# Genomics-GPU/Genomics-GPU

Hardware: AMD Instinct MI355X
Metric: GCUPS on batched 150bp affine-gap SW at 1/2/4/8 MI355X; HBM-roofline % (higher is better)
Workload: dtype int16x2 packed (exact value window), int32 fallback per declined block

## Files before the change

genomics-gpu_amd/csrc/dispatch.hip:

```cpp
#include <hip/hip_runtime.h>

#include <algorithm>
#include <cstdio>
#include <cstdlib>
#include <cstring>
#include <string>
#include <vector>

#include "banded16.hpp"
#include "local16.hpp"
#include "engine.hpp"
#include "generic.hpp"
#include "pairhmm.hpp"
#include "ksw16.hpp"
#include "start.hpp"
#include "wavefront.hpp"
#include "wavefront16.hpp"

namespace gx {

static thread_local std::string g_last_error;
void set_error(const std::string &msg) { g_last_error = msg; }
const char *last_error() { return g_last_error.c_str(); }

// ... 339 lines not shown
    uint32_t b0 = 0, p0 = 0, ppb = 1, lds_stride = 0;
    size_t lds_bytes = 0;
    int32_t vmin = 0;
};
static bool one_shape_only(const WfArgs &A) { return A.rev || A.n_dev || A.stop || A.lstop; }

static int device_cus(Workspace &ws) {
    if (!ws.cus) (void)hipDeviceGetAttribute(&ws.cus, hipDeviceAttributeMultiprocessorCount, ws.device);
    return ws.cus > 0 ? ws.cus : 256;
}

static TailShape tail_shape(Workspace &ws, const Plan &pl, const gasalx_params &p, const WfArgs &A, uint32_t n) {
    TailShape t;
    const bool on = env_flag("GASALX_TAIL", true);
    const int kextra = env_int("GASALX_TAIL_K", 0);
    if (!on || !pl.packed16 || (pl.tb && !pl.tb_band) || pl.key2 || pl.ku16 || pl.kseg_shift || pl.semi_tq ||
        one_shape_only(A))
        return t;
    int G2 = 0, R2 = 0;
    WfFn fn = nullptr;
    if (pl.wf_algo == WF_LOCAL && pl.kf16 && pl.G16 == 8 && pl.R16 == 19) {
        G2 = 32; R2 = 5; fn = &wf16_mix_kernel<WF_LOCAL, 8, 19, 32, 5>;
    } else if (pl.tb_band) {
        if (pl.wf_algo != WF_GLOBAL || pl.G16 != 16 || pl.R16 != 20) return t;
        if (env_int("GASALX_CP_TAIL", 64) == 32) {
            G2 = 32; R2 = 12; fn = &wf16_mix_kernel<WF16_GLOBAL_CP, 16, 20, 32, 12>;
        } else {
            G2 = 64; R2 = 8; fn = &wf16_mix_kernel<WF16_GLOBAL_CP, 16, 20, 64, 8>;
        }
    } else if (pl.wf_algo == WF_GLOBAL && pl.G16 == 16 && pl.R16 == 20) {
        G2 = 64; R2 = 5; fn = &wf16_mix_kernel<WF_GLOBAL, 16, 20, 64, 5>;
    } else {
        return t;
    }
    const int64_t q8 = pad8(pl.max_q), y8 = pad8(pl.max_t);
    if (pl.wf_algo == WF_LOCAL) {
        const LocalDrift d = local_drift_frame(p, q8, y8, G2, R2);
        if (!(d.window && d.f16)) return t;
        t.vmin = pl.vmin;
    } else {
        if (!packed16_ok(p, WF_GLOBAL, pl.max_q, pl.max_t, &t.vmin,
                         std::max(packed_span(G2, R2, y8), packed_span(pl.G16, pl.R16, y8))))
            return t;
        t.vmin = std::max(t.vmin, pl.vmin);
    }
    const uint64_t slots = (uint64_t)wf16_waves(pl.wf_algo, pl.R16) * 4 * device_cus(ws);
    const uint32_t ppw = pairs_per_wave(pl.G16), ppb = pairs_per_block(pl.G16);
    const uint64_t waves = (n + ppw - 1) / ppw;
    const uint64_t rounds = waves / slots;
    if (rounds < 2 + (uint64_t)std::max(kextra, 0)) return t;
    const uint64_t long_waves = (rounds - (uint64_t)std::max(kextra, 0)) * slots;
    t.b0 = (uint32_t)(long_waves / kWavesPerBlock);
    t.p0 = t.b0 * ppb;
    if (t.p0 >= n) return TailShape();
    t.ppb = pairs_per_block(G2);
    t.lds_stride = packed_lds_stride((uint32_t)y8, G2);
    t.lds_bytes = packed_lds_bytes((uint32_t)y8, G2);
    t.fn = fn;
    t.G2 = G2;
    t.R2 = R2;
    return t;
}

template <class Args>
static void fill_scoring(Args &A, const gasalx_params &p) {
    A.a = p.match; A.b = p.mismatch; A.o = p.gap_open; A.e = p.gap_extend;
    A.nval = p.n_code & 0xF;
    A.has_npen = p.has_n_penalty; A.npen = p.n_penalty;
}
static void wf_common(WfArgs &A, const gasalx_params &p, const Plan &pl) {
    fill_scoring(A, p);
    A.head = p.head; A.tail = p.tail;
    A.lds_stride = pl.lds_stride;
    A.force_exact = (p.mismatch <= 0 || (p.has_n_penalty && p.n_penalty < 0)) ? 1 : 0;
    A.one = 0x00010001u;
}

static int launch_int32(const Plan &pl, WfFn fn, const WfArgs &A, hipStream_t st) {
    if (!fn) { set_error("no wavefront instance"); return GASALX_EUNSUPPORTED; }
    HIPCHK(launch_lds(fn, dim3(wf_grid(A.n, pl.G, A.skip != nullptr)), dim3(kBlock), pl.lds_bytes, st, A));
    return GASALX_OK;
}

static int launch_wavefront(Workspace &ws, const Plan &pl, const gasalx_params &p, const WfArgs &base,
                            const TailShape &main_tail, hipStream_t st) {
    WfArgs A = base;
    const uint32_t n = A.n;
    wf_common(A, p, pl);
    if (pl.packed16) {
        WfArgs P16 = A;
        P16.lds_stride = pl.lds16_stride;
        P16.fast16 = 1;
        P16.vmin = pl.vmin;
        P16.kf16 = pl.kf16;
        const uint32_t ppb16 = pairs_per_block(pl.G16);
        uint32_t grid16 = grid_for(n, ppb16);
        const TailShape tail = one_shape_only(A) ? TailShape() : main_tail;
        size_t lds16 = pl.lds16_bytes;
        if (tail.fn) {
            P16.tail_b0 = tail.b0; P16.tail_p0 = tail.p0; P16.tail_lds = tail.lds_stride;
            P16.vmin = tail.vmin;
            grid16 = tail.b0 + grid_for(n - tail.p0, tail.ppb);
            lds16 = std::max(lds16, tail.lds_bytes);
        }
        HIPCHK(ws.misc.reserve(grid16 + 64));
        P16.handled = ws.misc.as<uint8_t>();
        ws.pk_flags = grid16; ws.pk_ppb = ppb16; ws.pk_pairs = n;
        ws.pk_p1 = tail.fn ? tail.p0 : 0xFFFFFFFFu; ws.pk_b1 = tail.b0; ws.pk_ppb2 = tail.fn ? tail.ppb : 1;
        if (pl.tb) {
            HIPCHK(ws.aux.reserve((size_t)n * 4));
            P16.tbfix = ws.aux.as<int32_t>();
        }
        Wf16Variant v;
        v.tb = pl.tb; v.tbd = pl.tb && pl.kf16 != 0;
        v.key2 = pl.key2; v.ku16 = pl.ku16; v.kseg = pl.kseg_shift != 0;
        v.lrs = pl.wf_algo == WF_LOCAL && !pl.tb && !pl.key2 && A.lstop != nullptr && pl.kf16 != 0 && !pl.kseg_shift;
        v.stop = A.stop != nullptr;
        WfFn f16 = pl.tb_band ? wf16_pick_r4<WF16_GLOBAL_CP>(pl.G16, pl.R16) : wf16_lookup(pl.wf_algo, pl.G16, pl.R16, v);
        if (A.rev && !pl.tb_band && (v.stop || v.lrs)) {
            const int ra = A.stop ? WF16_SEMI_STOP : pl.ku16 ? WF16_LOCAL_U16_RS : WF16_LOCAL_RS;
            if (WfFn rc = wf16_rclass_lookup(ra, pl.G16, pl.R16)) f16 = rc;
        }
        if (pl.kseg_shift) {
            const uint32_t nsave = std::max<uint32_t>(1u, (pl.kf16 + (uint32_t)pl.G16 - 2u) >> pl.kseg_shift);
            const uint64_t waves = (uint64_t)grid16 * kWavesPerBlock;
            HIPCHK(ws.kseg.reserve(waves * nsave * (uint64_t)pl.R16 * 64 * 4 + 64));
            P16.kseg = ws.kseg.as<uint32_t>();
            P16.kseg_shift = pl.kseg_shift;
            P16.kseg_n = nsave;
        }
        if (tail.fn) f16 = tail.fn;
        if (!f16) { set_error("no packed wavefront instance"); return GASALX_EUNSUPPORTED; }
        HIPCHK(launch_lds(f16, dim3(grid16), dim3(kBlock), lds16, st, P16));
        A.skip = ws.misc.as<uint8_t>();
        A.skip_ppb = ppb16;
        A.skip_p1 = tail.fn ? tail.p0 : 0xFFFFFFFFu;
        A.skip_b1 = tail.b0;
        A.skip_ppb2 = tail.fn ? tail.ppb : 1;
    }
    return launch_int32(pl, A.stop ? pick_instance<WfK<WF_SEMI, true, false, true>, SHAPES_R4>(pl.G, pl.R)
                                   : wf_lookup(pl.wf_algo, pl.keys, pl.tb && !pl.tb_band, pl.G, pl.R), A, st);
}

struct SortMeta {
    uint32_t *perm, *second, *hist, *cursor;
    size_t sh;
};
static int sort_reserve(Workspace &ws, uint32_t n, uint32_t nkeys, bool two, SortMeta *m) {
    m->sh = (size_t)(nkeys + 1) * 4;
    HIPCHK(ws.sort_meta.reserve((size_t)n * (two ? 8 : 4) + 2 * m->sh + 64));
    m->perm = ws.sort_meta.as<uint32_t>();
    m->second = two ? m->perm + n : nullptr;
    m->hist = m->perm + (two ? 2 : 1) * (size_t)n;
    m->cursor = m->hist + nkeys + 1;
    return GASALX_OK;
}
static int sort_histogram(const SortMeta &m, const uint32_t *keys, uint32_t n, uint32_t nkeys, hipStream_t st) {
    HIPCHK(hipMemsetAsync(m.hist, 0, m.sh, st));
    rev_hist_kernel<<<sort_grid(n), 256, m.sh, st>>>(REV_PLAIN, keys, nullptr, n, nkeys, m.hist);
    HIPCHK(hipGetLastError());
    return GASALX_OK;
}
static int sort_scatter(const SortMeta &m, const uint32_t *keys, uint32_t n, uint32_t nkeys, uint32_t *inv,
                        hipStream_t st) {
    rev_scan_kernel<<<1, 256, 0, st>>>(m.hist, m.cursor, nkeys + 1);
    rev_scatter_kernel<<<sort_grid(n), 256, 2 * m.sh, st>>>(REV_PLAIN, keys, nullptr, n, nkeys, m.cursor, m.perm, inv);
    HIPCHK(hipGetLastError());
    return GASALX_OK;
}
static int counting_sort(Workspace &ws, const uint32_t *keys, uint32_t n, uint32_t nkeys, hipStream_t st,
                         bool want_inv, const uint32_t **perm, const uint32_t **inv) {
    SortMeta m;
    int rc = sort_reserve(ws, n, nkeys, want_inv, &m);
    if (!rc) rc = sort_histogram(m, keys, n, nkeys, st);
    if (!rc) rc = sort_scatter(m, keys, n, nkeys, m.second, st);
    if (rc) return rc;
    *perm = m.perm;
    if (want_inv) *inv = m.second;
    return GASALX_OK;
}

static int launch_semi_tq(Workspace &ws, const Plan &pl, const gasalx_params &p, const WfArgs &base,
                          hipStream_t st, bool one_class) {
    WfArgs A = base;
    const uint32_t n = A.n;
    wf_common(A, p, pl);
    const uint32_t t8w = (uint32_t)pl.R16;
    SortMeta m;
    int rc = sort_reserve(ws, n, t8w, false, &m);
    if (rc) return rc;
    std::vector<uint32_t> h(t8w + 1, 0u);
    if (one_class) {
        h[0] = n;
    } else {
        if ((rc = sort_histogram(m, A.tlen, n, t8w, st))) return rc;
        HIPCHK(hipMemcpyAsync(h.data(), m.hist, m.sh, hipMemcpyDeviceToHost, st));
        HIPCHK(hipStreamSynchronize(st));
    }
    int classes = 0;
    for (uint32_t b = 0; b <= t8w; b++) classes += h[b] != 0;
    A.perm = nullptr;
    if (classes > 1) {
        if ((rc = sort_scatter(m, A.tlen, n, t8w, nullptr, st))) return rc;
        A.perm = m.perm;
    }
    HIPCHK(ws.misc.reserve(n + 64));
    HIPCHK(hipMemsetAsync(ws.misc.p, 0, n, st));
    ws.pk_flags = n; ws.pk_ppb = 1; ws.pk_pairs = n;
    WfArgs P16 = A;
    P16.lds_stride = pl.lds16_stride;
    P16.fast16 = 1;
    P16.vmin = pl.vmin;
    P16.handled = ws.misc.as<uint8_t>();
    const uint32_t ppb16 = pairs_per_block(8);
    uint32_t slot = 0;
    for (uint32_t b = 0; b <= t8w; slot += h[b], b++) {
// ... 611 lines not shown
```

genomics-gpu_amd/csrc/wavefront16.hpp:

```cpp
#pragma once
#include <hip/hip_runtime.h>
#include <stdint.h>

#include <type_traits>

#include "wavefront.hpp"

namespace gx {

typedef unsigned short pk_u2 __attribute__((ext_vector_type(2)));
#define GX_AS(T, x) __builtin_bit_cast(T, x)

__device__ __forceinline__ uint32_t pk_mad_u16(uint32_t a, uint32_t b, uint32_t c) {
    return GX_AS(uint32_t, GX_AS(pk_u2, a) * GX_AS(pk_u2, b) + GX_AS(pk_u2, c));
}
__device__ __forceinline__ uint32_t pk_mad_u16_lo(uint32_t a, uint32_t b, uint32_t c) {
    const pk_u2 cc = {(uint16_t)c, (uint16_t)c};
    return GX_AS(uint32_t, GX_AS(pk_u2, a) * GX_AS(pk_u2, b) + cc);
}
__device__ __forceinline__ uint32_t pk_max_u16(uint32_t a, uint32_t b) {
    return GX_AS(uint32_t, __builtin_elementwise_max(GX_AS(pk_u2, a), GX_AS(pk_u2, b)));
}
__device__ __forceinline__ uint32_t pk_addnc(uint32_t a, uint32_t b) { return a + b; }
__device__ __forceinline__ uint32_t pk_subnb(uint32_t a, uint32_t b) { return a - b; }
// ... 346 lines not shown
        Hout[k] = H;
    }
    f_out = f;
}

template <int R, int PV = 0>
__device__ __forceinline__ void step_semi(const uint2 T, const uint32_t diag_top, uint32_t &hl, uint32_t &el,
                                          const uint32_t (&xs)[R], const uint32_t (&Hin)[R], uint32_t (&Hout)[R],
                                          uint32_t (&Fk)[R], const uint32_t GO, const uint32_t *pv = nullptr) {
    uint32_t diag = diag_top, h = hl, e = el;
#pragma unroll
    for (int k = 0; k < R; ++k) {
        uint32_t v = __builtin_amdgcn_perm(T.y, T.x, xs[k]);
        if (PV > 0 && k >= R - PV) v = pk_addnc(v, pv[k - (R - PV)]);
        const uint32_t tmp = pk_addnc(diag, v);
        Fk[k] = pk_max_u16(Hin[k], Fk[k]);
        e = pk_max_u16(h, e);
        h = pk_subnb(pk_max3(tmp, Fk[k], e), GO);
        diag = Hin[k];
        Hout[k] = h;
    }
    hl = h;
    el = e;
}

template <int G, int R>
__device__ __forceinline__ void tb_store_window(const WfArgs &A, const uint32_t (&pr)[2], const bool (&valid)[2],
                                                const uint32_t (&W16)[2], const uint32_t w, const uint32_t lg,
                                                const uint32_t (&dw)[R]) {
    if (A.tb_q8) {
        if ((valid[0] && w < W16[0]) || (valid[1] && w < W16[1])) {
            uint4 *dst = reinterpret_cast<uint4 *>(A.tb + (uint64_t)(pr[0] & ~7u) * A.tb_pair_words) +
                         ((uint64_t)w * (R / 4) * G + lg) * 4 + ((pr[0] & 7u) >> 1);
#pragma unroll
            for (int k = 0; k < R; k += 4)
                dst[(k / 4) * G * 4] = make_uint4(__builtin_amdgcn_perm(dw[k + 1], dw[k], 0x05040100u),
                                                  __builtin_amdgcn_perm(dw[k + 3], dw[k + 2], 0x05040100u),
                                                  __builtin_amdgcn_perm(dw[k + 1], dw[k], 0x07060302u),
                                                  __builtin_amdgcn_perm(dw[k + 3], dw[k + 2], 0x07060302u));
        }
        return;
    }
#pragma unroll
    for (int h = 0; h < 2; ++h) {
        if (valid[h] && w < W16[h]) {
            uint16_t *dst = reinterpret_cast<uint16_t *>(A.tb + (uint64_t)pr[h] * A.tb_pair_words) +
                            (uint64_t)w * (G * R) + lg * 4;
            const uint32_t sel = h ? 0x07060302u : 0x05040100u;
#pragma unroll
            for (int k = 0; k < R; k += 4)
                *reinterpret_cast<uint2 *>(dst + k * G) =
                    make_uint2(__builtin_amdgcn_perm(dw[k + 1], dw[k], sel), __builtin_amdgcn_perm(dw[k + 3], dw[k + 2], sel));
        }
    }
}

constexpr int WF16_GLOBAL_TB = 3;
constexpr int WF16_LOCAL_TB = 4;
constexpr int WF16_LOCAL_K2 = 5;
constexpr int WF16_SEMI_TQ = 6;
__host__ __device__ constexpr uint32_t band_stream_words(uint32_t wd) { return ((wd + 1 + 3) & ~3u) + 8; }
constexpr int WF16_GLOBAL_CP = 7;
constexpr int WF16_SEMI_STOP = 9;
constexpr int WF16_LOCAL_U16 = 10;
constexpr int WF16_LOCAL_RS = 11;
constexpr int WF16_LOCAL_U16_RS = 12;
constexpr int WF16_LOCAL_SEG = 13;
constexpr int WF16_LOCAL_TBD = 14;
constexpr int kW16_LTBD_WAVES = 2;
constexpr int kW16_TQ_WAVES = 3;
constexpr int kW16_TQ_BIG_WAVES = 3;
constexpr int kW16_CP_WAVES = 3;

__host__ __device__ constexpr int wf16_waves(int algo, int R) {
    return algo == WF16_GLOBAL_TB ? kW16_TB_WAVES
           : algo == WF16_LOCAL_TB ? kW16_LTB_WAVES
           : algo == WF16_LOCAL_TBD ? kW16_LTBD_WAVES
           : algo == WF16_LOCAL_K2 ? kW16_K2_WAVES
           : algo == WF16_SEMI_TQ ? (R > 20 ? kW16_TQ_BIG_WAVES : kW16_TQ_WAVES)
           : algo == WF16_GLOBAL_CP ? kW16_CP_WAVES
           : GX_WF16_WAVES;
}

template <int ALGO_, int G, int R>
__global__ __launch_bounds__(kBlock, wf16_waves(ALGO_, R)) void wf16_kernel(WfArgs A) {
    const uint32_t wf16_bid = blockIdx.x, wf16_bl = blockIdx.x, wf16_p0 = 0, wf16_lds = A.lds_stride;
#include "wf16_body.inc"
}

template <int ALGO_, int G1, int R1, int G2, int R2>
__global__ __launch_bounds__(kBlock, wf16_waves(ALGO_, R1)) void wf16_mix_kernel(WfArgs A) {
    if (blockIdx.x < A.tail_b0) {
        constexpr int G = G1, R = R1;
        const uint32_t wf16_bid = blockIdx.x, wf16_bl = blockIdx.x, wf16_p0 = 0, wf16_lds = A.lds_stride;
#include "wf16_body.inc"
    } else {
        constexpr int G = G2, R = R2;
        const uint32_t wf16_bid = blockIdx.x, wf16_bl = blockIdx.x - A.tail_b0, wf16_p0 = A.tail_p0,
                       wf16_lds = A.tail_lds;
#include "wf16_body.inc"
    }
}

#define GX_SHAPES_R4(X) X(8, 8) X(8, 12) X(8, 16) X(8, 20) X(16, 16) X(16, 20) X(32, 20) X(64, 20)
#define GX_SHAPES_PK(X)                                                                               \
    X(8, 8) X(8, 12) X(8, 16) X(8, 19) X(8, 20) X(8, 23) X(16, 10) X(16, 12) X(16, 16) X(16, 20)      \
    X(32, 5) X(32, 6) X(32, 9) X(32, 20) X(64, 3) X(64, 5) X(64, 20)
enum ShapeSet { SHAPES_R4, SHAPES_PK };

template <class K, ShapeSet L>
auto pick_instance(int G, int R) -> decltype(K::template fn<8, 8>()) {
#define GX_CASE(g, r) if (G == g && R == r) return K::template fn<g, r>();
    if constexpr (L == SHAPES_R4) { GX_SHAPES_R4(GX_CASE) } else { GX_SHAPES_PK(GX_CASE) }
#undef GX_CASE
    return nullptr;
}

using Wf16Fn = void (*)(WfArgs);
template <int ALGO>
struct Wf16K {
    template <int G, int R> static Wf16Fn fn() { return &wf16_kernel<ALGO, G, R>; }
};

Wf16Fn wf16_tq_lookup(int R);
Wf16Fn wf16_local_lookup(int G, int R, bool u16, bool rs, bool seg = false);
Wf16Fn wf16_rclass_lookup(int algo, int G, int R);

}
```

genomics-gpu_amd/csrc/wf16_body.inc:

```
    extern __shared__ __attribute__((aligned(16))) uint8_t lds[];
    constexpr bool GTB = ALGO_ == WF16_GLOBAL_TB;
    constexpr bool GCP = ALGO_ == WF16_GLOBAL_CP;
    constexpr bool GT = GTB || GCP;
    constexpr bool LTB = ALGO_ == WF16_LOCAL_TB;
    constexpr bool K2 = ALGO_ == WF16_LOCAL_K2;
    constexpr bool KU16 = ALGO_ == WF16_LOCAL_U16 || ALGO_ == WF16_LOCAL_U16_RS;
    constexpr bool LRS = ALGO_ == WF16_LOCAL_RS || ALGO_ == WF16_LOCAL_U16_RS;
    constexpr bool KSEG = ALGO_ == WF16_LOCAL_SEG;
    constexpr bool LTBD = ALGO_ == WF16_LOCAL_TBD;
    constexpr bool TQ = ALGO_ == WF16_SEMI_TQ;
    static_assert(!TQ || G == 8, "TAIL=QUERY/BOTH instances are G = 8");
    constexpr bool STOPK = ALGO_ == WF16_SEMI_STOP;
    constexpr int ALGO = GT ? WF_GLOBAL : (LTB || K2 || KU16 || LRS || KSEG || LTBD) ? WF_LOCAL : (TQ || STOPK) ? WF_SEMI : ALGO_;
    constexpr int S = 64 / G;
    constexpr bool TR = ALGO == WF_SEMI;
    const uint32_t lane = threadIdx.x & 63, wave = threadIdx.x >> 6;
    const uint32_t lg = lane & (G - 1), slot = lane / G;
    const uint32_t nn = A.n_dev ? min(*A.n_dev > A.n_dev_off ? *A.n_dev - A.n_dev_off : 0u, A.n) : A.n;
    if (A.n_dev && wf16_p0 + wf16_bl * (uint32_t)(kWavesPerBlock * 2 * S) >= nn) return;
    const uint32_t wv = wf16_bl * kWavesPerBlock + wave;
    const uint32_t pair0 = (TQ ? A.slot0 : wf16_p0) + wv * (2 * S);
    const bool breg2 = GCP && wf16_p0 != 0;
    uint32_t *const bcp = breg2 ? A.cp2 : A.cp;
    uint2 *const bstm = breg2 ? A.stm2 : A.stm;
    uint4 *const bbfl = breg2 ? A.bflags2 : A.bflags;
    const uint32_t BWD = breg2 ? A.band_wd2 : A.band_wd;
    uint32_t pr[2], xl[2], yl[2], xo[2], yo[2], xpad[2], ypad[2];
    bool valid[2];
    const uint8_t *X = TR ? A.t : A.q, *Y = TR ? A.q : A.t;
#pragma unroll
    for (int h = 0; h < 2; ++h) {
        const uint32_t idx = pair0 + 2 * slot + h;
        valid[h] = idx < nn;
        pr[h] = (valid[h] && A.perm) ? A.perm[idx] : idx;
        const uint32_t ql = valid[h] ? A.qlen[pr[h]] : 0, tl = valid[h] ? A.tlen[pr[h]] : 0;
        const uint32_t qo = valid[h] ? A.qoff[pr[h]] : 0, to = valid[h] ? A.toff[pr[h]] : 0;
        xl[h] = TR ? tl : ql; yl[h] = TR ? ql : tl;
        xo[h] = TR ? to : qo; yo[h] = TR ? qo : to;
        xpad[h] = (xl[h] + 7u) & ~7u;
        ypad[h] = (yl[h] + 7u) & ~7u;
    }
    uint32_t ymaxw = max(ypad[0], ypad[1]);
#pragma unroll
    for (int m = 32; m >= 1; m >>= 1) ymaxw = max(ymaxw, (uint32_t)__shfl_xor(ymaxw, m));

    const Pk16 P = pk16_params<ALGO>(A);
    const int32_t NS = A.has_npen ? -A.npen : 0;
    const int32_t nrule = (ALGO == WF_GLOBAL) ? (A.has_npen ? NS : -A.b) : NS;
    const uint32_t t_mis = (uint32_t)(P.k - A.b) * 0x01010101u;
    const uint32_t t_n = (uint32_t)(nrule + P.k) * 0x01010101u;
    const uint32_t t_out = (uint32_t)P.k * 0x01010101u;
    const uint32_t t_match = (uint32_t)(A.a + P.k);

    const uint32_t words = wf16_lds >> 3;
    uint2 *wl = reinterpret_cast<uint2 *>(lds) + (size_t)wave * S * words;
    bool other = false;
    for (uint32_t base = 0; base < S * (words >> 2); base += 64) {
        const uint32_t idx = base + lane;
        const uint32_t ps = min(idx / (words >> 2), (uint32_t)S - 1);
        const uint32_t y0 = 4 * (idx - ps * (words >> 2)) - G;
        uint32_t tab[2][4];
#pragma unroll
        for (int h = 0; h < 2; ++h) {
            const uint32_t yp = __shfl(ypad[h], ps * G), yof = __shfl(yo[h], ps * G);
            const uint32_t ylen = __shfl(yl[h], ps * G);
            uint32_t v = 0;
            const bool in = (int32_t)y0 >= 0 && y0 < yp;
            if (in) v = load4_codes_dir(A, Y, yof, ylen, y0 >> 2);
#pragma unroll
            for (int j = 0; j < 4; ++j) {
                const uint32_t l = in ? letter_of((v >> (8 * j)) & 15u, A.nval) : 6u;
                other |= l == 5;
                if (GT && !A.has_npen) other |= l == 4 && y0 + j < ylen;
                if (GT) other |= in && y0 + j >= ylen && l != 4;
                tab[h][j] = l == 6 ? t_out : l == 4 ? t_n : (t_mis & ~(0xFFu << (8 * l))) | (t_match << (8 * l));
            }
        }
        if (idx < S * (words >> 2)) {
            uint2 *dst = wl + ps * words + 4 * (idx - ps * (words >> 2));
#pragma unroll
            for (int j = 0; j < 4; ++j) dst[j] = make_uint2(tab[0][j], tab[1][j]);
        }
    }
    const uint32_t r0 = lg * R;
    uint32_t xs[R];
#pragma unroll
    for (int k = 0; k < R; ++k) {
        const uint32_t r = r0 + k;
        xs[k] = 0x0C0C0C0Cu;
#pragma unroll
        for (int h = 0; h < 2; ++h) {
            if (valid[h] && r < xpad[h]) {
                const uint32_t pos = A.rev ? xl[h] - 1u - r : r;
                const uint32_t cde = A.rev && r >= xl[h] ? (uint32_t)A.nval
                                     : A.packed ? (load4_codes(X, xo[h], pos >> 2, 1) >> (8 * (pos & 3))) & 15u
                                                : (uint32_t)X[xo[h] + pos] & 15u;
                const uint32_t l = letter_of(cde, A.nval);
                if (r < xl[h]) {
                    other |= l >= 4;
                    xs[k] = (xs[k] & ~(0xFFu << (16 * h))) | ((l + 4 * h) << (16 * h));
                } else if (ALGO == WF_LOCAL || GT || TQ) {
                    other |= l != 4;
                }
            }
        }
    }
    constexpr int PV = TQ ? (R < 7 ? R : 7) : 0;
    uint32_t pv[PV > 0 ? PV : 1];
    if constexpr (TQ) {
        const int32_t nrule = A.has_npen ? -A.npen : 0;
#pragma unroll
        for (int j = 0; j < PV; ++j) {
            const uint32_t r = r0 + (R - PV) + j;
            pv[j] = 0;
#pragma unroll
            for (int h = 0; h < 2; ++h)
                if (valid[h] && r >= xl[h] && r < xpad[h]) pv[j] |= (uint32_t)(nrule + P.k) << (16 * h);
        }
#pragma unroll
        for (int h = 0; h < 2; ++h) other |= valid[h] && xpad[h] != (uint32_t)(G * R);
    } else {
#pragma unroll
        for (int h = 0; h < 2; ++h) other |= valid[h] && xpad[h] > (uint32_t)(G * R);
    }
    const bool fast = A.fast16 && !A.force_exact && !__syncthreads_or(other);
    if constexpr (TQ) {
        if (lg == 0)
#pragma unroll
            for (int h = 0; h < 2; ++h)
                if (valid[h]) A.handled[pair0 + 2 * slot + h] = fast ? 1 : 0;
    } else if (threadIdx.x == 0) {
        A.handled[wf16_bid] = fast ? 1 : 0;
    }
    if (!fast) return;

    const uint32_t nsteps = ymaxw + G - 1;
    const uint2 *tcol = wl + slot * words;
    const uint32_t EXT = pk_bcast(A.e);
    const uint32_t GO = pk_bcast(A.o);
    const uint32_t BB = (uint32_t)P.base * 0x10001u;
    const uint32_t NN = (uint32_t)P.neg * 0x10001u;
    const bool top = lg == 0;
    int32_t c = -(int32_t)lg;

    auto band_pass = [&]() __attribute__((always_inline)) {
      if constexpr (GCP) {
        static_assert(R % 4 == 0, "band windows store flags in groups of 4 rows");
        const int32_t pb = P.base, go = A.o, ge = A.e, D = P.drift;
        const uint32_t KX = pk_bcast(P.k - 2 * D), OEX = pk_bcast(P.k - 2 * D + A.o + A.e - D);
        const uint32_t WD = BWD;
        const int32_t L = max((int32_t)r0 - (int32_t)A.band_w, 0);
        uint32_t HA[R], HB[R], Ek[R], dw[R];
        const uint32_t *cpw = bcp + ((size_t)wv * 64 + lane) * (2 * R);
#pragma unroll
        for (int k = 0; k < R; ++k) {
            const int32_t r = (int32_t)r0 + k;
            HA[k] = L == 0 ? (uint32_t)(pb + D * (r - 1) - (r <= 0 ? 0 : go + ge * r)) * 0x10001u : cpw[k];
            Ek[k] = L == 0 ? NN : cpw[R + k];
            HB[k] = HA[k];
            dw[k] = 0;
        }
        const uint32_t SW = band_stream_words(WD);
        const uint4 *sp = reinterpret_cast<const uint4 *>(bstm + ((size_t)wv * 64 + (lane ? lane - 1 : 0)) * SW);
        uint4 B0a = sp[0], B0b = sp[1], B1a = sp[2], B1b = sp[3];
        if (L == 0) B0a.x = (uint32_t)(pb + D * ((int32_t)r0 - 2) - (r0 <= 1 ? 0 : go + ge * ((int32_t)r0 - 1))) * 0x10001u;
        uint4 *bf = bbfl + ((size_t)wv * 64 + lane) * (WD / 4) * (R / 4);
        const bool any = valid[0] || valid[1];
        c = L;
        uint32_t fdummy = NN;
        auto bstep = [&](const int j, uint32_t (&Hin)[R], uint32_t (&Hout)[R], const uint32_t hd, const uint32_t fu)
            __attribute__((always_inline)) {
            const uint2 T = tcol[c + G];
            const uint32_t dtop = (uint32_t)(pb + D * (c - 2) - (c <= 0 ? 0 : go + ge * c)) * 0x10001u;
            step_global_tb<R, true>(T, top ? dtop : hd, top ? NN : fu, xs, Hin, Hout, Ek, dw, fdummy, KX, OEX, NN, j);
            ++c;
        };
        const uint32_t tmax = (uint32_t)L <= ymaxw ? min(WD, (ymaxw + 1u - (uint32_t)L + 3u) & ~3u) : 0u;
        for (uint32_t t = 0; t < WD; t += 4) {
            if (t >= tmax) break;
            const uint4 B2a = sp[t / 2 + 4], B2b = sp[t / 2 + 5];
            bstep(0, HA, HB, B0a.x, B0a.w);
            bstep(1, HB, HA, B0a.z, B0b.y);
            bstep(2, HA, HB, B0b.x, B0b.w);
            bstep(3, HB, HA, B0b.z, B1a.y);
            B0a = B1a; B0b = B1b; B1a = B2a; B1b = B2b;
            if (any) {
                uint4 *dst = bf + (t / 4) * (R / 4);
#pragma unroll
                for (int k = 0; k < R; k += 4)
                    dst[k / 4] = make_uint4(__builtin_amdgcn_perm(dw[k + 1], dw[k], 0x05040100u),
                                            __builtin_amdgcn_perm(dw[k + 3], dw[k + 2], 0x05040100u),
                                            __builtin_amdgcn_perm(dw[k + 1], dw[k], 0x07060302u),
                                            __builtin_amdgcn_perm(dw[k + 3], dw[k + 2], 0x07060302u));
            }
        }
      }
    };

    if (ALGO == WF_LOCAL) {
        const uint32_t KK = pk_bcast(P.k), OEK = pk_bcast(A.o + A.e + P.k);
        const uint32_t KMUL = A.one << 8;
        const uint32_t bshift = ((uint32_t)P.base << 8) & 0xFFFFu;
        uint32_t HA[R], HB[R], Ek[R], key[R], key2[K2 ? R : 1];
        uint32_t jseg = 0;
#pragma unroll
        for (int k = 0; k < R; ++k) { HA[k] = BB; HB[k] = BB; Ek[k] = BB; key[k] = 0; }
#pragma unroll
        for (int k = 0; k < (K2 ? R : 1); ++k) key2[k] = 0;
        uint32_t recvH = BB, prevRecvH = BB, recvF = BB, f = BB;
        uint2 tnext = tcol[c + G];
        if constexpr (LTB) {
            static_assert(R % 4 == 0, "LOCAL+TB packed shapes need R % 4 == 0");
            uint32_t dw[R];
#pragma unroll
            for (int k = 0; k < R; ++k) dw[k] = 0;
            uint32_t W16[2];
#pragma unroll
// ... 75 lines not shown
#pragma unroll
                    for (int h = 0; h < 2; ++h) sstop[h] = valid[h] ? A.lstop[pr[h]] : 0;
                }
                if constexpr (LTBD) {
                    static_assert(R % 4 == 0, "LOCAL+TB packed shapes need R % 4 == 0");
                    uint32_t dw[R];
#pragma unroll
                    for (int k = 0; k < R; ++k) dw[k] = 0;
                    uint32_t W16[2];
#pragma unroll
                    for (int h = 0; h < 2; ++h) W16[h] = (ypad[h] + G + 2) >> 2;
                    uint32_t FL0 = FL[0];
                    auto tstep = [&](auto keysc, const int j, uint32_t (&Hin)[R], uint32_t (&Hout)[R])
                        __attribute__((always_inline)) {
                        constexpr bool KEYS = decltype(keysc)::value;
                        const uint2 T = tnext;
                        tnext = tcol[c + j + 1 + G];
                        const uint32_t dt = (uint32_t)(pbv + ge * (c + j - 2)) * 0x10001u;
                        step_local_tb_dr<R, KEYS, KA0T>(T, top ? dt : prevRecvH, top ? BB : recvF, xs, Hin, Hout, Ek, key, FL0,
                                                  dw, f, KXD, OEXD, EXT, KMV, KEYS ? inv(s + j - 1, 0) : 0u,
                                                  KEYS ? inv(s + j, (uint32_t)(-ge)) : 0u, EXT2, MK, j);
                        prevRecvH = recvH;
                        recvH = pk_subnb((uint32_t)shr_lane((int32_t)Hout[R - 1]), ADJV);
                        recvF = pk_subnb((uint32_t)shr_lane((int32_t)f), ADJV);
                    };
                    for (; s < nsteps; s += 4, c += 4) {
                        tstep(std::false_type{}, 0, HA, HB);
                        tstep(std::true_type{}, 1, HB, HA);
                        tstep(std::false_type{}, 2, HA, HB);
                        tstep(std::true_type{}, 3, HB, HA);
                        tb_store_window<G, R>(A, pr, valid, W16, s >> 2, lg, dw);
                    }
                }
                for (; !LTBD && s < nsteps; s += 2, c += 2) {
                    if (KSEG && s == segend && jseg < A.kseg_n) {
                        uint32_t *dst = A.kseg + (((size_t)wv * A.kseg_n + jseg) * 64 + lane) * R;
#pragma unroll
                        for (int k = 0; k < R; ++k) { dst[k] = key[k]; key[k] = KOFS * 0x10001u; }
                        ++jseg;
                        segend += MK;
                    }
                    uint2 T = tnext;
                    tnext = tcol[c + 1 + G];
                    const uint32_t dt0 = (uint32_t)(pbv + ge * (c - 2)) * 0x10001u;
                    step_local_dr<R, false, KU16>(T, top ? dt0 : prevRecvH, top ? BB : recvF, xs, HA, HB, Ek, key, FL, f,
                                            KXD, OEXD, EXT, KMC, 0u, 0u, EXT2);
                    prevRecvH = recvH;
                    recvH = pk_subnb((uint32_t)shr_lane((int32_t)HB[R - 1]), ADJV);
                    recvF = pk_subnb((uint32_t)shr_lane((int32_t)f), ADJV);
                    T = tnext;
                    tnext = tcol[c + 2 + G];
                    const uint32_t dt1 = (uint32_t)(pbv + ge * (c - 1)) * 0x10001u;
                    step_local_dr<R, true, KU16, KA0>(T, top ? dt1 : prevRecvH, top ? BB : recvF, xs, HB, HA, Ek, key, FL,
                                                    f, KXD, OEXD, EXT, KMV, inv(s, 0), inv(s + 1, (uint32_t)(-ge)), EXT2, MK);
                    prevRecvH = recvH;
                    recvH = pk_subnb((uint32_t)shr_lane((int32_t)HA[R - 1]), ADJV);
                    recvF = pk_subnb((uint32_t)shr_lane((int32_t)f), ADJV);
                    if (LRS && (s & 7u) == 6u) {
                        const int32_t cl = (int32_t)s + 1 - (G - 1);
                        const int32_t m = min(((cl + 1) & ~7) - 1, (int32_t)C - 1);
                        if (m >= 0) {
                            uint32_t mx = key[0];
#pragma unroll
                            for (int k = 1; k < R; ++k) mx = pk_max_u16(mx, key[k]);
                            bool hit[2];
#pragma unroll
                            for (int h = 0; h < 2; ++h) {
                                const uint32_t thr = KOFS + (uint32_t)sstop[h] * MK +
                                                     (CP - 1u - (uint32_t)m - lg);
                                hit[h] = !valid[h] || sstop[h] <= 0 || ((mx >> (16 * h)) & 0xFFFFu) >= thr;
                            }
                            if (groups_all<G>(__ballot(hit[0])) && groups_all<G>(__ballot(hit[1]))) break;
                        }
                    }
                }
                if constexpr (KA0 || KA0T) {
#pragma unroll
                    for (int k = 1; k < R; ++k) key[k] -= (((uint32_t)(ge * k) * MK) & 0xFFFFu) * 0x10001u;
                }
            } else {
                sweep(std::integral_constant<int, 0>{}, nsteps);
            }
        }
        uint64_t bestv[2] = {0, 0};
        static_assert(R <= 32, "row index of the merge codes: 5 bits");
        const bool fastkey = !K2 && !LTB && !KSEG && A.kf16 && A.kf16 + G <= 2048;
        if (fastkey) {
            const uint32_t C = A.kf16 + G;
            constexpr uint32_t KOFS_ = KU16 ? 0u : 0x0400u;
            uint32_t km = key[0];
#pragma unroll
            for (int k = 1; k < R; ++k) km = pk_max_u16(km, key[k]);
            uint32_t thr = 0, Hm[2];
#pragma unroll
            for (int h = 0; h < 2; ++h) {
                Hm[h] = (((km >> (16 * h)) & 0xFFFFu) - KOFS_) / C;
                thr |= (KOFS_ + Hm[h] * C) << (16 * h);
            }
            const uint32_t cb = pk_bcast((int32_t)(C - 1u - lg));
            const pk_u2 one = {1, 1}, ffff = {0xFFFF, 0xFFFF};
            uint32_t bc = 0xFFFFFFFFu;
#pragma unroll
            for (int k = 0; k < R; ++k) {
                const uint32_t t = GX_AS(uint32_t, GX_AS(pk_u2, key[k]) - GX_AS(pk_u2, thr));
                const pk_u2 below = __builtin_elementwise_min(__builtin_elementwise_sub_sat(GX_AS(pk_u2, thr),
                                                                                            GX_AS(pk_u2, key[k])), one);
                const uint32_t col = GX_AS(uint32_t, GX_AS(pk_u2, cb) - GX_AS(pk_u2, t));
                const pk_u2 sh5 = {5, 5};
                const uint32_t code = GX_AS(uint32_t, GX_AS(pk_u2, col & 0xFFF8FFF8u) << sh5) | (col & 0x00070007u) |
                                      ((uint32_t)(k << 3) * 0x10001u) | GX_AS(uint32_t, below * ffff);
                bc = GX_AS(uint32_t, __builtin_elementwise_min(GX_AS(pk_u2, bc), GX_AS(pk_u2, code)));
            }
#pragma unroll
            for (int h = 0; h < 2; ++h) {
                const uint32_t c16 = (bc >> (16 * h)) & 0xFFFFu, k = (c16 >> 3) & 31u, r = r0 + k;
                if (Hm[h] > 0 && c16 != 0xFFFFu && r < xpad[h]) {
                    const uint32_t ord = (((c16 >> 8) * xpad[h] + r) << 3) + (c16 & 7u);
                    bestv[h] = ((uint64_t)Hm[h] << 32) | (0xFFFFFFFFu - ord);
                }
            }
        }
#pragma unroll
        for (int h = 0; h < 2; ++h) {
            uint64_t best = bestv[h];
#pragma unroll
            for (int k = 0; k < R && !fastkey; ++k) {
                const uint32_t r = r0 + k;
                const uint32_t kk = (key[k] >> (16 * h)) & 0xFFFFu;
                uint32_t H = kk >> 8, col = 255u - (kk & 0xFFu);
                if (KSEG) {
                    const uint32_t ms = A.kseg_shift;
                    H = 0;
                    col = 0;
                    auto seg = [&](const uint32_t j, const uint32_t kv) __attribute__((always_inline)) {
                        const uint32_t x = ((kv >> (16 * h)) & 0xFFFFu) - 0x0400u;
                        const uint32_t Hj = x >> ms, t = x & ((1u << ms) - 1u);
                        if (Hj > H) { H = Hj; col = ((j + 1) << ms) - 1u - t - lg; }
                    };
                    const uint32_t *src = A.kseg + ((size_t)wv * A.kseg_n * 64 + lane) * R + k;
                    for (uint32_t j = 0; j < jseg; ++j) seg(j, src[(size_t)j * (64 * R)]);
                    seg(jseg, key[k]);
                }
                if constexpr (K2) {
                    const uint32_t k2v = (key2[k] >> (16 * h)) & 0xFFFFu;
                    if ((k2v >> 8) > H) { H = k2v >> 8; col = 511u - (k2v & 0xFFu); }
                }
                if (r < xpad[h] && H > 0) {
                    const uint32_t ord = (((col >> 3) * xpad[h] + r) << 3) + (col & 7);
                    const uint64_t cand = ((uint64_t)H << 32) | (0xFFFFFFFFu - ord);
                    best = cand > best ? cand : best;
                }
            }
            best = group_max_u64<G>(best);
            if (valid[h] && lg == 0) {
                int32_t H = (int32_t)(best >> 32), qe = 0, te = 0;
                if (H > 0) {
                    const uint32_t ord = 0xFFFFFFFFu - (uint32_t)best;
                    const uint32_t rest = ord >> 3;
                    qe = (int32_t)(rest % xpad[h]);
                    te = (int32_t)((rest / xpad[h]) * 8 + (ord & 7));
                }
                A.score[pr[h]] = H;
                if (A.qend) A.qend[pr[h]] = qe;
                if (A.tend) A.tend[pr[h]] = te;
            }
        }
    } else if (ALGO == WF_GLOBAL) {
        const int32_t pb = P.base, go = A.o, ge = A.e, D = P.drift;
        const uint32_t KX = pk_bcast(P.k - 2 * D), OEX = pk_bcast(P.k - 2 * D + A.o + A.e - D);
        auto left = [=](int32_t r) -> uint32_t {
            return (uint32_t)(pb + D * (r - 1) - (r <= 0 ? 0 : go + ge * r)) * 0x10001u;
        };
        const uint32_t L_0 = (uint32_t)(pb - D) * 0x10001u, L_in = (uint32_t)(pb - D - go) * 0x10001u;
        uint32_t HA[R], HB[R], Ek[R];
        uint32_t dw[GTB ? R : 1];
#pragma unroll
        for (int k = 0; k < R; ++k) { HA[k] = left((int32_t)(r0 + k)); HB[k] = HA[k]; Ek[k] = NN; }
#pragma unroll
        for (int k = 0; k < (GTB ? R : 1); ++k) dw[k] = 0;
        uint32_t recvH = left((int32_t)r0 - 1), prevRecvH = recvH, recvF = NN, f = NN;
        uint32_t kq_lane[2], kq[2], kp_lane[2], kp[2];
        bool fixable[2];
        int32_t score[2] = {0, 0}, fixv[2] = {0, 0};
#pragma unroll
        for (int h = 0; h < 2; ++h) {
            kq_lane[h] = (xl[h] - 1) / R;
            kq[h] = (xl[h] - 1) - kq_lane[h] * R;
            fixable[h] = GT && valid[h] && xl[h] < xpad[h] && yl[h] < ypad[h];
            kp_lane[h] = xl[h] / R;
            kp[h] = xl[h] - kp_lane[h] * R;
        }
        const int32_t cs_own = GCP ? max((int32_t)r0 - (int32_t)A.band_w, 0) - 1 : -1;
        const int32_t cs_dn = GCP ? max((int32_t)(r0 + R) - (int32_t)A.band_w, 0) - 1 : 0;
        const bool cp_on = GCP && (valid[0] || valid[1]);
        const bool st_on = cp_on && lg + 1 < G;
        uint32_t *cpw = GCP ? bcp + ((size_t)wv * 64 + lane) * (2 * R) : nullptr;
        uint2 *stw = GCP ? bstm + ((size_t)wv * 64 + lane) * band_stream_words(BWD) : nullptr;
        uint2 tnext = tcol[c + G];
        uint32_t cap_lo = 0xFFFFFFFFu, cap_hi = 0;
#pragma unroll
        for (int h = 0; h < 2; ++h) {
            if (valid[h]) {
                const uint32_t sq = yl[h] - 1 + kq_lane[h];
                cap_lo = min(cap_lo, sq);
                cap_hi = max(cap_hi, sq);
                if (fixable[h]) {
                    const uint32_t sf = yl[h] + kp_lane[h];
                    cap_lo = min(cap_lo, sf);
                    cap_hi = max(cap_hi, sf);
                }
            }
        }
#pragma unroll
        for (int m = 32; m >= 1; m >>= 1) {
            cap_lo = min(cap_lo, (uint32_t)__shfl_xor(cap_lo, m));
            cap_hi = max(cap_hi, (uint32_t)__shfl_xor(cap_hi, m));
        }
        auto half_step = [&](auto flg, const int32_t cc, const int j, uint32_t (&Hin)[R], uint32_t (&Hout)[R]) __attribute__((always_inline)) {
            constexpr int FLG = decltype(flg)::value;
            const uint2 T = tnext;
            tnext = tcol[cc + 1 + G];
            if ((FLG & 1) && cc == -1) {
#pragma unroll
                for (int k = 0; k < R; ++k) { Hout[k] = k == 0 && r0 == 0 ? L_0 : L_in; Ek[k] = NN; }
                f = NN;
                if (GTB && j == 0) {
#pragma unroll
                    for (int k = 0; k < R; ++k) dw[k] = 0;
                }
            } else {
                const uint32_t dtop = (uint32_t)(pb + D * (cc - 2) - (cc <= 0 ? 0 : go + ge * cc)) * 0x10001u;
                if constexpr (GTB)
                    step_global_tb<R>(T, top ? dtop : prevRecvH, top ? NN : recvF, xs, Hin, Hout, Ek, dw, f, KX,
                                      OEX, NN, j);
                else
                    step_global<R, GCP>(T, top ? dtop : prevRecvH, top ? NN : recvF, xs, Hin, Hout, Ek, f, KX, OEX, NN);
                if constexpr ((FLG & 2) != 0) {
#pragma unroll
                    for (int h = 0; h < 2; ++h) {
                        if (valid[h] && cc == (int32_t)yl[h] - 1 && lg == kq_lane[h]) {
                            uint32_t v = 0;
#pragma unroll
                            for (int k = 0; k < R; ++k) v = (k == (int)kq[h]) ? Hout[k] : v;
                            score[h] = (int32_t)((v >> (16 * h)) & 0xFFFFu) - pb - D * (int32_t)(xl[h] + yl[h] - 2);
                        }
                        if (fixable[h] && cc == (int32_t)yl[h] && lg == kp_lane[h]) {
                            uint32_t v = 0;
#pragma unroll
                            for (int k = 0; k < R; ++k) v = (k == (int)kp[h]) ? Hout[k] : v;
// ... 196 lines not shown
```

Before: 7366.

## Batch target-profile loads and pre-fetch query codes as dwords in local wf16 kernel

For the local-alignment packed16 kernel, the LDS profile build now issues up to six rounds of global code loads before consuming any of them, so more memory requests are in flight at once. Query codes for each lane's rows are read as aligned dwords and shifted with alignbyte instead of being loaded byte by byte. Metadata loads for invalid pairs are clamped to the last valid pair so they are issued unconditionally. It also adds optional wall-clock stamp instrumentation, compiled only under a macro. The trade-off is higher register pressure from the staged fetch buffers.

```diff
diff --git a/genomics-gpu_amd/csrc/dispatch.hip b/genomics-gpu_amd/csrc/dispatch.hip
--- a/genomics-gpu_amd/csrc/dispatch.hip
+++ b/genomics-gpu_amd/csrc/dispatch.hip
@@ -445,6 +445,33 @@
     return GASALX_OK;
 }
 
+#ifdef GX_WF16_STAMP
+static hipError_t stamp_begin(uint32_t waves, unsigned long long **buf) {
+    *buf = nullptr;
+    if (!std::getenv("GASALX_STAMP_OUT")) return hipSuccess;
+    hipError_t e = hipMalloc((void **)buf, (size_t)waves * 5 * 8);
+    if (e == hipSuccess) e = hipMemset(*buf, 0, (size_t)waves * 5 * 8);
+    if (e == hipSuccess) e = hipMemcpyToSymbol(HIP_SYMBOL(gx_wf16_stamp), buf, sizeof *buf);
+    return e;
+}
+static hipError_t stamp_end(uint32_t waves, unsigned long long *buf, hipStream_t st) {
+    if (!buf) return hipSuccess;
+    std::vector<unsigned long long> h((size_t)waves * 5);
+    unsigned long long *none = nullptr;
+    hipError_t e = hipStreamSynchronize(st);
+    if (e == hipSuccess) e = hipMemcpy(h.data(), buf, h.size() * 8, hipMemcpyDeviceToHost);
+    if (e == hipSuccess) e = hipMemcpyToSymbol(HIP_SYMBOL(gx_wf16_stamp), &none, sizeof none);
+    (void)hipFree(buf);
+    if (e == hipSuccess) {
+        if (FILE *f = std::fopen(std::getenv("GASALX_STAMP_OUT"), "wb")) {
+            std::fwrite(h.data(), 8, h.size(), f);
+            std::fclose(f);
+        }
+    }
+    return e;
+}
+#endif
+
 static int launch_wavefront(Workspace &ws, const Plan &pl, const gasalx_params &p, const WfArgs &base,
                             const TailShape &main_tail, hipStream_t st) {
     WfArgs A = base;
@@ -494,7 +521,14 @@
         }
         if (tail.fn) f16 = tail.fn;
         if (!f16) { set_error("no packed wavefront instance"); return GASALX_EUNSUPPORTED; }
+#ifdef GX_WF16_STAMP
+        unsigned long long *stamps = nullptr;
+        HIPCHK(stamp_begin(grid16 * kWavesPerBlock, &stamps));
+#endif
         HIPCHK(launch_lds(f16, dim3(grid16), dim3(kBlock), lds16, st, P16));
+#ifdef GX_WF16_STAMP
+        HIPCHK(stamp_end(grid16 * kWavesPerBlock, stamps, st));
+#endif
         A.skip = ws.misc.as<uint8_t>();
         A.skip_ppb = ppb16;
         A.skip_p1 = tail.fn ? tail.p0 : 0xFFFFFFFFu;
diff --git a/genomics-gpu_amd/csrc/wavefront16.hpp b/genomics-gpu_amd/csrc/wavefront16.hpp
--- a/genomics-gpu_amd/csrc/wavefront16.hpp
+++ b/genomics-gpu_amd/csrc/wavefront16.hpp
@@ -452,6 +452,17 @@
            : GX_WF16_WAVES;
 }
 
+#ifdef GX_WF16_STAMP
+static __device__ unsigned long long *gx_wf16_stamp;
+#define GX_WF16_STAMP_AT(i)                                                               \
+    do {                                                                                  \
+        if (gx_wf16_stamp && lane == 0)                                                   \
+            gx_wf16_stamp[((size_t)wf16_bid * kWavesPerBlock + wave) * 5 + (i)] = wall_clock64(); \
+    } while (0)
+#else
+#define GX_WF16_STAMP_AT(i) do { } while (0)
+#endif
+
 template <int ALGO_, int G, int R>
 __global__ __launch_bounds__(kBlock, wf16_waves(ALGO_, R)) void wf16_kernel(WfArgs A) {
     const uint32_t wf16_bid = blockIdx.x, wf16_bl = blockIdx.x, wf16_p0 = 0, wf16_lds = A.lds_stride;
diff --git a/genomics-gpu_amd/csrc/wf16_body.inc b/genomics-gpu_amd/csrc/wf16_body.inc
--- a/genomics-gpu_amd/csrc/wf16_body.inc
+++ b/genomics-gpu_amd/csrc/wf16_body.inc
@@ -19,6 +19,13 @@
     const uint32_t nn = A.n_dev ? min(*A.n_dev > A.n_dev_off ? *A.n_dev - A.n_dev_off : 0u, A.n) : A.n;
     if (A.n_dev && wf16_p0 + wf16_bl * (uint32_t)(kWavesPerBlock * 2 * S) >= nn) return;
     const uint32_t wv = wf16_bl * kWavesPerBlock + wave;
+    GX_WF16_STAMP_AT(0);
+#ifdef GX_WF16_STAMP
+    if (gx_wf16_stamp && lane == 0)
+        gx_wf16_stamp[((size_t)wf16_bid * kWavesPerBlock + wave) * 5 + 4] =
+            (unsigned long long)__builtin_amdgcn_s_getreg((31 << 11) | 4) |
+            ((unsigned long long)__builtin_amdgcn_s_getreg((31 << 11) | 20) << 32);
+#endif
     const uint32_t pair0 = (TQ ? A.slot0 : wf16_p0) + wv * (2 * S);
     const bool breg2 = GCP && wf16_p0 != 0;
     uint32_t *const bcp = breg2 ? A.cp2 : A.cp;
@@ -32,9 +39,15 @@
     for (int h = 0; h < 2; ++h) {
         const uint32_t idx = pair0 + 2 * slot + h;
         valid[h] = idx < nn;
-        pr[h] = (valid[h] && A.perm) ? A.perm[idx] : idx;
-        const uint32_t ql = valid[h] ? A.qlen[pr[h]] : 0, tl = valid[h] ? A.tlen[pr[h]] : 0;
-        const uint32_t qo = valid[h] ? A.qoff[pr[h]] : 0, to = valid[h] ? A.toff[pr[h]] : 0;
+        const uint32_t ic = ALGO_ == WF_LOCAL ? min(idx, nn - 1u) : idx;
+        pr[h] = ((ALGO_ == WF_LOCAL || valid[h]) && A.perm) ? A.perm[ic] : ic;
+    }
+#pragma unroll
+    for (int h = 0; h < 2; ++h) {
+        const bool ld = ALGO_ == WF_LOCAL || valid[h];
+        uint32_t ql = ld ? A.qlen[pr[h]] : 0, tl = ld ? A.tlen[pr[h]] : 0;
+        uint32_t qo = ld ? A.qoff[pr[h]] : 0, to = ld ? A.toff[pr[h]] : 0;
+        if (!valid[h]) ql = tl = qo = to = 0;
         xl[h] = TR ? tl : ql; yl[h] = TR ? ql : tl;
         xo[h] = TR ? to : qo; yo[h] = TR ? qo : to;
         xpad[h] = (xl[h] + 7u) & ~7u;
@@ -55,18 +68,49 @@
     const uint32_t words = wf16_lds >> 3;
     uint2 *wl = reinterpret_cast<uint2 *>(lds) + (size_t)wave * S * words;
     bool other = false;
-    for (uint32_t base = 0; base < S * (words >> 2); base += 64) {
-        const uint32_t idx = base + lane;
-        const uint32_t ps = min(idx / (words >> 2), (uint32_t)S - 1);
-        const uint32_t y0 = 4 * (idx - ps * (words >> 2)) - G;
+    constexpr bool BATCH = ALGO_ == WF_LOCAL;
+    constexpr int kFetch = BATCH ? 6 : 1;
+    const uint32_t r0 = lg * R;
+    constexpr int XW = (R + 3) / 4;
+    const bool xdw = BATCH && !A.packed && !A.rev;
+    uint32_t xd[2][XW + 1];
+    if (xdw) {
+#pragma unroll
+        for (int h = 0; h < 2; ++h)
+#pragma unroll
+            for (int i = 0; i <= XW; ++i) {
+                const uint32_t w = (r0 >> 2) + i;
+                xd[h][i] = valid[h] && 4 * w < xpad[h] ? reinterpret_cast<const uint32_t *>(X + xo[h])[w] : 0u;
+            }
+    }
+    const uint32_t nquad = S * (words >> 2);
+    for (uint32_t base = 0; base < nquad; base += 64 * kFetch) {
+      uint32_t fps[kFetch], fy0[kFetch], fv[kFetch][2];
+#pragma unroll
+      for (int t = 0; t < kFetch; ++t) {
+        if (t && base + 64 * t >= nquad) continue;
+        const uint32_t idx = base + 64 * t + lane;
+        fps[t] = min(idx / (words >> 2), (uint32_t)S - 1);
+        fy0[t] = 4 * (idx - fps[t] * (words >> 2)) - G;
+#pragma unroll
+        for (int h = 0; h < 2; ++h) {
+            const uint32_t yp = __shfl(ypad[h], fps[t] * G), yof = __shfl(yo[h], fps[t] * G);
+            const uint32_t ylen = __shfl(yl[h], fps[t] * G);
+            fv[t][h] = 0;
+            if ((int32_t)fy0[t] >= 0 && fy0[t] < yp) fv[t][h] = load4_codes_dir(A, Y, yof, ylen, fy0[t] >> 2);
+        }
+      }
+#pragma unroll
+      for (int t = 0; t < kFetch; ++t) {
+        if (t && base + 64 * t >= nquad) continue;
+        const uint32_t idx = base + 64 * t + lane, ps = fps[t], y0 = fy0[t];
         uint32_t tab[2][4];
 #pragma unroll
         for (int h = 0; h < 2; ++h) {
-            const uint32_t yp = __shfl(ypad[h], ps * G), yof = __shfl(yo[h], ps * G);
+            const uint32_t yp = __shfl(ypad[h], ps * G);
             const uint32_t ylen = __shfl(yl[h], ps * G);
-            uint32_t v = 0;
+            const uint32_t v = fv[t][h];
             const bool in = (int32_t)y0 >= 0 && y0 < yp;
-            if (in) v = load4_codes_dir(A, Y, yof, ylen, y0 >> 2);
 #pragma unroll
             for (int j = 0; j < 4; ++j) {
                 const uint32_t l = in ? letter_of((v >> (8 * j)) & 15u, A.nval) : 6u;
@@ -76,14 +120,20 @@
                 tab[h][j] = l == 6 ? t_out : l == 4 ? t_n : (t_mis & ~(0xFFu << (8 * l))) | (t_match << (8 * l));
             }
         }
-        if (idx < S * (words >> 2)) {
+        if (idx < nquad) {
             uint2 *dst = wl + ps * words + 4 * (idx - ps * (words >> 2));
 #pragma unroll
             for (int j = 0; j < 4; ++j) dst[j] = make_uint2(tab[0][j], tab[1][j]);
         }
-    }
-    const uint32_t r0 = lg * R;
+      }
+    }
     uint32_t xs[R];
+    if (xdw) {
+#pragma unroll
+        for (int h = 0; h < 2; ++h)
+#pragma unroll
+            for (int i = 0; i < XW; ++i) xd[h][i] = __builtin_amdgcn_alignbyte(xd[h][i + 1], xd[h][i], r0 & 3u);
+    }
 #pragma unroll
     for (int k = 0; k < R; ++k) {
         const uint32_t r = r0 + k;
@@ -92,7 +142,8 @@
         for (int h = 0; h < 2; ++h) {
             if (valid[h] && r < xpad[h]) {
                 const uint32_t pos = A.rev ? xl[h] - 1u - r : r;
-                const uint32_t cde = A.rev && r >= xl[h] ? (uint32_t)A.nval
+                const uint32_t cde = xdw ? (xd[h][k / 4] >> (8 * (k & 3))) & 15u
+                                     : A.rev && r >= xl[h] ? (uint32_t)A.nval
                                      : A.packed ? (load4_codes(X, xo[h], pos >> 2, 1) >> (8 * (pos & 3))) & 15u
                                                 : (uint32_t)X[xo[h] + pos] & 15u;
                 const uint32_t l = letter_of(cde, A.nval);
@@ -133,6 +184,7 @@
         A.handled[wf16_bid] = fast ? 1 : 0;
     }
     if (!fast) return;
+    GX_WF16_STAMP_AT(1);
 
     const uint32_t nsteps = ymaxw + G - 1;
     const uint2 *tcol = wl + slot * words;
@@ -374,6 +426,7 @@
                 sweep(std::integral_constant<int, 0>{}, nsteps);
             }
         }
+        GX_WF16_STAMP_AT(2);
         uint64_t bestv[2] = {0, 0};
         static_assert(R <= 32, "row index of the merge codes: 5 bits");
         const bool fastkey = !K2 && !LTB && !KSEG && A.kf16 && A.kf16 + G <= 2048;
@@ -457,6 +510,7 @@
                 if (A.tend) A.tend[pr[h]] = te;
             }
         }
+        GX_WF16_STAMP_AT(3);
     } else if (ALGO == WF_GLOBAL) {
         const int32_t pb = P.base, go = A.o, ge = A.e, D = P.drift;
         const uint32_t KX = pk_bcast(P.k - 2 * D), OEX = pk_bcast(P.k - 2 * D + A.o + A.e - D);
```

After: 7582, median of 6. 2.9% higher.
